# rmcar17/SpectralClusterSupertree

Hardware: AMD Instinct MI355X
Metric: top-level PCG build + Fiedler solve wall-time (s) at N taxa, 1/2/4/8 MI355X (lower is better)
Workload: dtype f64 (loop operator: fp32 image of W; fp64 renewal + confirmation)

## Files before the change

spectralclustersupertree_amd/csrc/scs_build.hip:

```cpp

#include <algorithm>

#include "scs_internal.h"

typedef unsigned long long u64;
typedef unsigned int u32;

constexpr u32 DEPTH_INF = 0xFFFFFFFFu;


__device__ __forceinline__ void rmq_offsets(int m, int a, int b, int (&o)[2]) {
    const int k = 31 - __clz(b - a);
    o[0] = k * m + a;
    o[1] = k * m + b - (1 << k);
}

template <typename K>
__device__ __forceinline__ K rmq_min(const K *__restrict__ base, int m, int a, int b) {
    int o[2];
    rmq_offsets(m, a, b, o);
    const K x = base[o[0]], y = base[o[1]];
    return x < y ? x : y;
}

// ... 1109 lines not shown
        SCS_HIP_CHECK(hipEventSynchronize(ev_x.b));
        SCS_HIP_CHECK(hipEventElapsedTime(&exch_ms, ev_x.a, ev_x.b));
        exch_bytes = (double)chunk_doubles * 8.0 * (world - 1);
    } else if (shared) {
        std::vector<int32_t> splits;
        SCS_TRY(scs_gather_row_splits(ctx, row_begin, row_end, n, splits));
        auto needs = [&](int dst, const int2 &t) {
            const int64_t lo = splits[dst], hi = splits[dst + 1];
            const int64_t r_lo = (int64_t)t.x * SCS_TR, r_hi = std::min<int64_t>(r_lo + SCS_TR, n);
            const int64_t c_lo = (int64_t)t.y * cols_per_tile, c_hi = std::min<int64_t>(c_lo + cols_per_tile, n);
            return (r_lo < hi && lo < r_hi) || (c_lo < hi && lo < c_hi);
        };
        std::vector<int64_t> send_off(world + 1, 0), recv_off(world + 1, 0);
        std::vector<int32_t> send_slots;
        std::vector<int2> recv_tiles;
        for (int p = 0; p < world; ++p) {
            for (size_t i = rank; i < all_tiles.size(); i += world)
                if (needs(p, all_tiles[i])) send_slots.push_back((int32_t)(i / world));
            send_off[p + 1] = (int64_t)send_slots.size() * SCS_TR * cols_per_tile;
            for (size_t i = p; i < all_tiles.size(); i += world)
                if (needs(rank, all_tiles[i])) recv_tiles.push_back(all_tiles[i]);
            recv_off[p + 1] = (int64_t)recv_tiles.size() * SCS_TR * cols_per_tile;
        }
        cached_buf d_send(ctx), d_recv(ctx);
        dev_buf d_slots(ctx), d_rtiles(ctx);
        SCS_TRY(d_send.alloc((size_t)send_off[world] * 8));
        SCS_TRY(d_recv.alloc((size_t)recv_off[world] * 8));
        SCS_TRY(d_slots.alloc(send_slots.size() * 4));
        SCS_TRY(d_rtiles.alloc(recv_tiles.size() * sizeof(int2)));
        ev_pair ev_x;
        SCS_TRY(ev_x.init());
        SCS_HIP_CHECK(hipEventRecord(ev_x.a, s));
        SCS_HIP_CHECK(hipMemcpyAsync(d_slots.p, send_slots.data(), send_slots.size() * 4,
                                     hipMemcpyHostToDevice, s));
        SCS_HIP_CHECK(hipMemcpyAsync(d_rtiles.p, recv_tiles.data(), recv_tiles.size() * sizeof(int2),
                                     hipMemcpyHostToDevice, s));
        if (!send_slots.empty())
            k_pack_tiles<<<(unsigned)send_slots.size(), 256, 0, s>>>(
                (const double *)d_tile_out.p, (const int32_t *)d_slots.p, cols_per_tile, (double *)d_send.p);
        SCS_HIP_CHECK(hipGetLastError());
        SCS_TRY(scs_comm_alltoallv_f64(&ctx->comm, (const double *)d_send.p, send_off.data(),
                                       (double *)d_recv.p, recv_off.data(), s));
        if (!recv_tiles.empty())
            k_unpack_received<<<(unsigned)recv_tiles.size(), cols_per_tile, 0, s>>>(
                (const double *)d_recv.p, (const int2 *)d_rtiles.p, n, row_begin, row_end, g->d_w,
                g->ld);
        SCS_HIP_CHECK(hipGetLastError());
        SCS_HIP_CHECK(hipEventRecord(ev_x.b, s));
        SCS_HIP_CHECK(hipEventSynchronize(ev_x.b));
        SCS_HIP_CHECK(hipEventElapsedTime(&exch_ms, ev_x.a, ev_x.b));
        exch_bytes = (double)(recv_off[world] - (recv_off[rank + 1] - recv_off[rank])) * 8.0;
    }
    SCS_HIP_CHECK(hipEventRecord(ev_total.b, s));
    SCS_HIP_CHECK(hipEventSynchronize(ev_total.b));
    h_off.in_flight = false;
    SCS_TRY(scs_tables_finish(ctx, tb));
    float total_ms = 0.f;
    SCS_HIP_CHECK(hipEventElapsedTime(&total_ms, ev_total.a, ev_total.b));
    if (n_batches == 1) {
        SCS_HIP_CHECK(hipEventElapsedTime(&prep_ms, ev_prep.a, ev_prep.b));
        SCS_HIP_CHECK(hipEventElapsedTime(&acc_ms, ev_acc.a, ev_acc.b));
        if (single_batch_spec) spec_ms = acc_ms;
    }

    if (stats) {
        memset(stats, 0, sizeof(*stats));
        stats->n_taxa = n;
        stats->n_trees = M;
        stats->row_begin = row_begin;
        stats->row_end = row_end;
        stats->symmetric = shared ? 2 : (sym ? 1 : 0);
        stats->exchange_ms = exch_ms;
        stats->exchange_bytes = exch_bytes;
        stats->n_tiles = (int32_t)tiles.size();
        stats->n_batches = n_batches;
        stats->spec_batches = spec_batches;
        stats->tree_parallel_batches = tree_par ? n_batches : 0;
        stats->spec_trees = spec_trees;
        stats->listed_batches = listed_batches;
        stats->prep_pieces = prep_pieces;
        stats->spec_ms = spec_ms;
        stats->cell_trees = (double)tiles.size() * SCS_TR * cols_per_tile * (double)M;
        stats->prep_ms = prep_ms;
        stats->accumulate_ms = acc_ms;
        stats->total_ms = total_ms;
        stats->bytes_w = 8.0 * rows * (double)n;
        stats->bytes_tables = 16.0 * (double)tb->n_leaves + 8.0 * M;
    }
    gd.g = nullptr;
    *out = g;
    return SCS_OK;
}

extern "C" int scs_graph_contract(scs_ctx *ctx, scs_graph *g, const int32_t *group_start,
                                  int32_t n_groups, scs_graph **out) {
    SCS_REQUIRE(ctx && g && group_start && out, "scs_graph_contract: null argument");
    if (g->mf) {
        scs_set_error("scs_graph_contract: a matrix-free graph has no matrix to contract");
        return SCS_EUNSUP;
    }
    if (g->upper) {
        scs_set_error("scs_graph_contract: an SCS_BUILD_UPPER graph holds no whole rows; build it "
                      "row-partitioned (SCS_BUILD_SHARED) when the node contracts");
        return SCS_EUNSUP;
    }
    SCS_REQUIRE(n_groups >= 1 && n_groups <= g->n, "scs_graph_contract: bad group count %d",
// ... 30 lines not shown
    if (e != hipSuccess) {
        scs_graph_free(ctx, ng);
        scs_set_error("scs_graph_contract: kernel failed: %s", hipGetErrorString(e));
        return SCS_EHIP;
    }
    scs_graph_free(ctx, g);
    *out = ng;
    return SCS_OK;
}

extern "C" int scs_graph_download_rows(scs_ctx *ctx, const scs_graph *g, int32_t first, int32_t count,
                                       double *out);

extern "C" int scs_graph_download(scs_ctx *ctx, const scs_graph *g, double *out) {
    SCS_REQUIRE(ctx && g && out, "scs_graph_download: null argument");
    SCS_REQUIRE(!g->mf, "scs_graph_download: a matrix-free graph has no matrix");
    SCS_HIP_CHECK(hipSetDevice(ctx->device));
    SCS_HIP_CHECK(hipStreamSynchronize(ctx->stream));
    const size_t rows = (size_t)(g->row_end - g->row_begin);
    if (g->upper) return scs_graph_download_rows(ctx, g, g->row_begin, (int32_t)rows, out);
    SCS_HIP_CHECK(hipMemcpy2D(out, (size_t)g->n * 8, g->d_w, (size_t)g->ld * 8, (size_t)g->n * 8,
                              rows, hipMemcpyDeviceToHost));
    return SCS_OK;
}

extern "C" int scs_graph_download_rows(scs_ctx *ctx, const scs_graph *g, int32_t first,
                                       int32_t count, double *out) {
    SCS_REQUIRE(ctx && g && out, "scs_graph_download_rows: null argument");
    SCS_REQUIRE(!g->mf, "scs_graph_download_rows: a matrix-free graph has no matrix");
    SCS_REQUIRE(count >= 1 && first >= g->row_begin && first + count <= g->row_end,
                "scs_graph_download_rows: rows [%d, %d) outside this rank's block [%d, %d)", first,
                first + count, g->row_begin, g->row_end);
    SCS_HIP_CHECK(hipSetDevice(ctx->device));
    SCS_HIP_CHECK(hipStreamSynchronize(ctx->stream));
    if (g->upper) {
        const size_t wcols = (size_t)(g->n - g->col0);
        for (int32_t i = 0; i < count; ++i) memset(out + (size_t)i * g->n, 0, (size_t)g->n * 8);
        SCS_HIP_CHECK(hipMemcpy2D(out + g->col0, (size_t)g->n * 8,
                                  g->d_w + (int64_t)(first - g->row_begin) * g->ld, (size_t)g->ld * 8,
                                  wcols * 8, (size_t)count, hipMemcpyDeviceToHost));
        for (int32_t i = 0; i < count; ++i) {
            const int32_t c0 = (first + i) / 256 * 256;
            if (c0 > g->col0) memset(out + (size_t)i * g->n + g->col0, 0, (size_t)(c0 - g->col0) * 8);
        }
        return SCS_OK;
    }
    SCS_HIP_CHECK(hipMemcpy2D(out, (size_t)g->n * 8, g->d_w + (int64_t)(first - g->row_begin) * g->ld,
                              (size_t)g->ld * 8, (size_t)g->n * 8, (size_t)count,
                              hipMemcpyDeviceToHost));
    return SCS_OK;
}

int scs_graph_prepare_degrees_begin(scs_ctx *ctx, scs_graph *g, bool want_w32) {
    if (g->deg_stage) return SCS_OK;
    const int n = g->n;
    const int rows = g->row_end - g->row_begin;
    if (g->mf && !g->have_deg) {
        SCS_HIP_CHECK(hipSetDevice(ctx->device));
        hipStream_t s = ctx->stream;
        if (!g->d_deg) SCS_TRY(scs_block_alloc(ctx, (size_t)n * 8, (void **)&g->d_deg));
        if (!g->d_dinv) SCS_TRY(scs_block_alloc(ctx, (size_t)n * 8, (void **)&g->d_dinv));
        SCS_TRY(scs_matfree_apply(ctx, g, nullptr, 0, 4, nullptr, s));
        k_dinv<<<(n + 255) / 256, 256, 0, s>>>(g->d_deg, n, g->d_dinv);
        SCS_HIP_CHECK(hipGetLastError());
        SCS_TRY(scs_pinned_get(ctx, (size_t)n * 8, &g->deg_stage));
        SCS_HIP_CHECK(hipMemcpyAsync(g->deg_stage, g->d_deg, (size_t)n * 8, hipMemcpyDeviceToHost, s));
        return SCS_OK;
    }
    const bool img_rows = ctx->comm.world > 1 && !g->upper;
    bool need_img = want_w32 && !g->have_w32 && !g->upper &&
                    (img_rows || (ctx->comm.world == 1 && g->row_begin == 0 && rows == n));
    if (g->have_deg && !need_img) return SCS_OK;
    SCS_HIP_CHECK(hipSetDevice(ctx->device));
    hipStream_t s = ctx->stream;
    if (need_img && !g->d_w32) {
        const size_t need = (size_t)rows * g->ld * 4;
        std::lock_guard<std::mutex> lock(ctx->cache_mu);
        if (ctx->w32_cache && ctx->w32_cache_bytes >= need) {
            g->d_w32 = ctx->w32_cache;
            g->w32_bytes = ctx->w32_cache_bytes;
            ctx->w32_cache = nullptr;
            ctx->w32_cache_bytes = 0;
        } else if (scs_dev_malloc(ctx, (void **)&g->d_w32, need) == hipSuccess) {
            g->w32_bytes = need;
            if (scs_dbg("SCS_TRACE_SOLVES") && atoi(scs_dbg("SCS_TRACE_SOLVES")))
                fprintf(stderr, "[image] hipMalloc of %.2f GB\n", need / 1073741824.0);
        } else {
            (void)hipGetLastError();
            g->d_w32 = nullptr;
            need_img = false;
        }
    }
    if (!need_img && g->have_deg) return SCS_OK;
    if (need_img && img_rows && g->have_deg) {
        dev_buf tmp(ctx);
        SCS_TRY(tmp.alloc((size_t)n * 8));
        k_degrees<true><<<(rows + 3) / 4, 256, 0, s>>>(g->d_w, g->ld, n, rows, g->row_begin, (double *)tmp.p, g->d_w32, 1);
        SCS_HIP_CHECK(hipGetLastError());
        SCS_HIP_CHECK(hipStreamSynchronize(s));
        g->have_w32 = true;
        return SCS_OK;
    }
    if (!g->d_deg) SCS_TRY(scs_block_alloc(ctx, (size_t)n * 8, (void **)&g->d_deg));
    if (!g->d_dinv) SCS_TRY(scs_block_alloc(ctx, (size_t)n * 8, (void **)&g->d_dinv));
    const int world = ctx->comm.world;
    if (need_img && !img_rows) {
        k_degrees<true><<<(rows + 3) / 4, 256, 0, s>>>(g->d_w, g->ld, n, rows, g->row_begin, g->d_deg, g->d_w32);
// ... 185 lines not shown
```

spectralclustersupertree_amd/csrc/scs_eig.hip:

```cpp

#include <algorithm>
#include <chrono>
#include <cmath>

#include "scs_internal.h"
#include "scs_policy.h"
#include "scs_symm.h"
#include "scs_matfree.h"
#include "scs_symm_tri.h"

#include <sched.h>
#include "scs_panel.h"

constexpr int MAXB = 16;
constexpr int MAXS = 64;
constexpr int SLD = MAXS + 1;

typedef double v4d __attribute__((ext_vector_type(4)));

__global__ void k_scale_rows(const double *__restrict__ x, int ldx, int c0, int b, int n,
                             const double *__restrict__ dinv, double *__restrict__ zt,
                             int64_t ldz) {
    const int idx = blockIdx.x * blockDim.x + threadIdx.x;
    if (idx >= n * b) return;
// ... 1595 lines not shown
        bool armed = false;
        double drop_tol = 0.0, seq = 0.0;
        double *report = nullptr;
    } tf1;
    dbuf coef1;
    bool use32 = false;
    bool gram_from32 = false;
    int n_apply32 = 0;
    std::vector<char> ev32;
    const double *fold_u = nullptr;
    int *fold_mask_r = nullptr;
    const double *fold_theta = nullptr;
    size_t ypart_cap = 0;
    int64_t chunk = 0;
    int gram_blocks = 0;
    std::vector<int32_t> splits;
    std::vector<hipEvent_t> ev;
    std::vector<hipEvent_t> ev_ag;
    hipEvent_t ev_cal[2] = {nullptr, nullptr};
    bool time_ag = false;
    int n_allgather = 0;
    int n_apply = 0;

    ~solver() {
        if (ctx) {
            ctx->event_pool.insert(ctx->event_pool.end(), ev.begin(), ev.end());
            ctx->event_pool.insert(ctx->event_pool.end(), ev_ag.begin(), ev_ag.end());
            for (auto e : ev_cal)
                if (e) ctx->event_pool.push_back(e);
        } else {
            for (auto e : ev_cal)
                if (e) hipEventDestroy(e);
            for (auto e : ev) hipEventDestroy(e);
            for (auto e : ev_ag) hipEventDestroy(e);
        }
    }
    int new_event(hipEvent_t *e) {
        if (ctx && !ctx->event_pool.empty()) {
            *e = ctx->event_pool.back();
            ctx->event_pool.pop_back();
            return SCS_OK;
        }
        SCS_HIP_CHECK(hipEventCreate(e));
        return SCS_OK;
    }

    double *small_at(int off) const { return small.d() + off; }

    void bind(scs_ctx *c, int n_, int b_ = 0, scs_graph *g_ = nullptr) {
        ctx = c;
        g = g_;
        s = c->stream;
        n = n_;
        b = b_;
        rows = g ? g->row_end - g->row_begin : 0;
        world = c->comm.world;
        gram_blocks = 256;
    }
    int team_splits() {
        SCS_TRY(scs_gather_row_splits(ctx, g->row_begin, g->row_end, g->n, splits));
        int max_rows = 0;
        for (int r = 0; r < world; ++r) max_rows = std::max(max_rows, splits[r + 1] - splits[r]);
        chunk = g->upper ? (int64_t)n * b : (int64_t)max_rows * b;
        return SCS_OK;
    }
    int team_buffers() {
        if (world == 1 || part_mode) return SCS_OK;
        SCS_TRY(yfull.alloc((size_t)n * b * 8));
        SCS_TRY(recv.alloc((size_t)chunk * world * 8));
        SCS_TRY(splits_d.alloc((size_t)(world + 1) * 4));
        SCS_HIP_CHECK(hipMemcpyAsync(splits_d.p, splits.data(), (size_t)(world + 1) * 4, hipMemcpyHostToDevice, s));
        return SCS_OK;
    }

    static bool image_layout(const scs_ctx *ctx, const scs_graph *g, int b) {
        const int world = ctx->comm.world;
        const bool one = world == 1 && !g->upper && g->row_begin == 0 && g->row_end == g->n;
        const bool row_ranks = world > 1 && !g->upper;
        return !g->mf && g->n >= 4096 && b == 4 && (one || row_ranks);
    }

    int gather(const double *send, double *recvb, size_t count) {
        hipEvent_t a = nullptr, b = nullptr;
        if (time_ag) {
            SCS_TRY(new_event(&a));
            SCS_TRY(new_event(&b));
            ev_ag.push_back(a);
            ev_ag.push_back(b);
            SCS_HIP_CHECK(hipEventRecord(a, s));
        }
        SCS_TRY(scs_comm_allgather_f64(&ctx->comm, send, recvb, count, s));
        if (time_ag) SCS_HIP_CHECK(hipEventRecord(b, s));
        ++n_allgather;
        return SCS_OK;
    }

    int last_nseg = 1;

    bool tri = false, part_mode = false;
    int tri_ct = 2, tri_nct = 0, tri_ntiles = 0;
    int tri_rb_lo = 0, tri_rb_hi = 0x7FFFFFFF;
    bool tri_backwards = false;
    dbuf tri_tiles, tri_pdir, tri_ptr, ysend;
    std::vector<int2> tiles_host;
    int tri32_nct = 0, tri32_ntiles = 0;
    double w32_bytes_per_apply = 0.0;
    int64_t ldz = 0;
    double w_bytes_per_apply = 0.0;

    int launch_symm_tri(const double *zin, double *yout) {
        const int tw = tri_ct * 128;
        const double *w_eff = g->d_w - (int64_t)g->row_begin * g->ld - g->col0;
        double *ptr_eff = tri_ptr.d() - (int64_t)tri_rb_lo * n * b;
        const int n_tf = panel_blocks16();
        const int ntiles = use32 ? tri32_ntiles : tri_ntiles;
#define TRI_T(B_, CT_, RPW_, D_, WT_, W_)                                                            \
    if (tf1.armed)                                                                                   \
        k_symm_tri_tf<B_, CT_, RPW_, D_, WT_><<<ntiles + n_tf, 256, 0, s>>>(                         \
            W_, g->ld, n, zin, ldz, tile_list, tri_pdir.d(), ptr_eff, n_tf, q.d(), fold_u,           \
            part.d(), n_tf, tf1.drop_tol, fold_mask_r, fold_theta, tf1.report, tf1.seq, part2.d(),   \
            coef1.d());                                                                              \
    else                                                                                             \
        k_symm_tri<B_, CT_, RPW_, D_, WT_><<<ntiles, 256, 0, s>>>(W_, g->ld, n, zin, ldz,            \
                                                                      tile_list, tri_pdir.d(), ptr_eff)
#define TRI(B_, CT_, RPW_, D_) TRI_T(B_, CT_, RPW_, D_, double, w_eff)
        const int2 *tile_list = (const int2 *)tri_tiles.p + (use32 ? 2 * tri_ntiles : 0) + (tri_backwards ? ntiles : 0);
        tri_backwards = !tri_backwards;
        if (use32) {
            TRI_T(4, 2, 2, 3, float, g->d_w32);
            ++n_apply32;
        } else if (b == 4) {
            if (tri_ct == 4) TRI(4, 4, 2, 3);
            else if (tri_ct == 1) TRI(4, 1, 4, 4);
            else TRI(4, 2, 4, 3);
        } else {
            if (tri_ct == 1) TRI(8, 1, 2, 6);
            else TRI(8, 2, 2, 4);
        }
#undef TRI
#undef TRI_T
        SCS_HIP_CHECK(hipGetLastError());
        tf1.armed = false;
        const bool img_tiles = use32;
        if (part_mode) {
            k_symm_tri_finish<<<(4 * n * b + 255) / 256, 256, 0, s>>>(tri_pdir.d(), ptr_eff, n, b, tw, tri_nct,
                                                                  nullptr, ysend.d(), tri_rb_lo, tri_rb_hi);
            SCS_HIP_CHECK(hipGetLastError());
            SCS_TRY(gather(ysend.d(), recv.d(), (size_t)n * b));
            if (yout) {
                k_sum_parts<<<(n * b + 255) / 256, 256, 0, s>>>(recv.d(), world, n, b, g->d_dinv, yout);
                SCS_HIP_CHECK(hipGetLastError());
            }
            last_nseg = world;
            return SCS_OK;
        }
        k_symm_tri_finish<<<(4 * n * b + 255) / 256, 256, 0, s>>>(tri_pdir.d(), tri_ptr.d(), n, b, img_tiles ? 512 : tw,
                                                              img_tiles ? tri32_nct : tri_nct,
                                                              yout ? g->d_dinv : nullptr,
                                                              yout ? yout : ypart.d());
        SCS_HIP_CHECK(hipGetLastError());
        last_nseg = 1;
        return SCS_OK;
    }
// ... 9 lines not shown
            return SCS_OK;
        }
        if (tri) return launch_symm_tri(zin, yout);
        const int64_t ld = g->ld;
        int rpw = 4, sdepth = 2;
        if (b == 16) rpw = 2;
        if (b == 4) sdepth = 4;
        const int rowblocks = (rows + 4 * rpw - 1) / (4 * rpw);
        const int n_macros = (int)(ld / (sdepth * SYMM_SUB));
        int nseg = (1024 + rowblocks - 1) / rowblocks;
        nseg = std::max(1, std::min(std::min(nseg, 4), n_macros));
        if (b == 8 && nseg < 2 && n_macros >= 2 && rowblocks < 2048) nseg = 2;
        const int mps = (n_macros + nseg - 1) / nseg;
        nseg = (n_macros + mps - 1) / mps;
        if (ypart_cap < (size_t)nseg * rows * b) {
            scs_set_error("internal: ypart buffer too small");
            return SCS_EINVAL;
        }
        dim3 grid((unsigned)rowblocks, (unsigned)nseg);
        switch (b) {
            case 4:
                if (use32) {
                    ++n_apply32;
                    k_symm<4, 4, 4, 3, float><<<grid, 256, 0, s>>>(g->d_w32, ld, rows, zin, ypart.d(), mps);
                } else {
                    k_symm<4, 4, 4, 3><<<grid, 256, 0, s>>>(g->d_w, ld, rows, zin, ypart.d(), mps);
                }
                break;
            case 8:
                k_symm<8, 4, 2, 2><<<grid, 256, 0, s>>>(g->d_w, ld, rows, zin, ypart.d(), mps);
                break;
            case 12:
                k_symm<12, 4, 2, 1><<<grid, 256, 0, s>>>(g->d_w, ld, rows, zin, ypart.d(), mps);
                break;
            case 16:
                k_symm<16, 2, 2, 2><<<grid, 256, 0, s>>>(g->d_w, ld, rows, zin, ypart.d(), mps);
                break;
            default:
                scs_set_error("unsupported block width %d (need 4, 8, 12 or 16)", b);
                return SCS_EUNSUP;
        }
        SCS_HIP_CHECK(hipGetLastError());
        last_nseg = nseg;
        if (yout)
            k_symm_finish<<<(rows * b + 255) / 256, 256, 0, s>>>(ypart.d(), nseg, rows, b,
                                                                 g->d_dinv, g->row_begin, yout);
        return SCS_OK;
    }

    int alloc_symm_buffers() {
        ypart_cap = (size_t)4 * rows * b;
        SCS_TRY(ypart.alloc(ypart_cap * 8));
        ldz = g->upper ? scs_round_up(n, SCS_LD_ALIGN) : g->ld;
        SCS_TRY(z.alloc((size_t)b * ldz * 8));
        SCS_HIP_CHECK(hipMemsetAsync(z.p, 0, (size_t)b * ldz * 8, s));
        w_bytes_per_apply = 8.0 * rows * (double)n;
        w32_bytes_per_apply = 4.0 * rows * (double)n;
        if (g->mf)
            w_bytes_per_apply = 2.0 * 16.0 * (double)g->mf->tb->n_leaves +
                                2.0 * 2.0 * 8.0 * (double)g->mf->tb->n_trees * (double)n * b;
        if (g->upper) {
            if (b != 4 && b != 8) {
                scs_set_error("an SCS_BUILD_UPPER graph is solved with block width 4 or 8 (asked: %d)", b);
                return SCS_EUNSUP;
            }
            tri = true;
            part_mode = true;
            tri_ct = 2;
            const int tw = 256;
            tri_nct = (n + tw - 1) / tw;
            tri_rb_lo = g->row_begin / TRI_TH;
            tri_rb_hi = (g->row_end + TRI_TH - 1) / TRI_TH;
            std::vector<int2> tiles;
            for (int i = tri_rb_lo; i < tri_rb_hi; ++i)
                for (int j = i * TRI_TH / tw; j < tri_nct; ++j) tiles.push_back(make_int2(i, j));
            tri_ntiles = (int)tiles.size();
            tiles.insert(tiles.end(), tiles.rbegin(), tiles.rend());
            SCS_TRY(tri_tiles.alloc(std::max<size_t>(tiles.size(), 1) * sizeof(int2)));
            SCS_HIP_CHECK(hipMemcpyAsync(tri_tiles.p, tiles.data(), tiles.size() * sizeof(int2),
                                         hipMemcpyHostToDevice, s));
            SCS_HIP_CHECK(hipStreamSynchronize(s));
            SCS_TRY(tri_pdir.alloc((size_t)tri_nct * n * b * 8));
            SCS_TRY(tri_ptr.alloc((size_t)(tri_rb_hi - tri_rb_lo) * n * b * 8));
            SCS_TRY(ysend.alloc((size_t)n * b * 8));
            if (!recv.p) SCS_TRY(recv.alloc((size_t)n * b * world * 8));
            w_bytes_per_apply = 8.0 * (double)tri_ntiles * TRI_TH * tw;
            return SCS_OK;
        }
        tri = !g->mf && world == 1 && rows == n && g->row_begin == 0 && n >= 4096 && (b == 4 || b == 8);
        if (tri) {
            const int tw = tri_ct * 128;
            const int n_rb = (n + TRI_TH - 1) / TRI_TH;
            tri_nct = (n + tw - 1) / tw;
            std::vector<int2> &tiles = tiles_host;
            tiles.clear();
            for (int i = 0; i < n_rb; ++i)
                for (int j = i * TRI_TH / tw; j < tri_nct; ++j) tiles.push_back(make_int2(i, j));
            tri_ntiles = (int)tiles.size();
            tiles.insert(tiles.end(), tiles.rbegin(), tiles.rend());
            {
                std::vector<int2> t32;
                tri32_nct = (n + 511) / 512;
                for (int i = 0; i < n_rb; ++i)
                    for (int j = i * TRI_TH / 512; j < tri32_nct; ++j) t32.push_back(make_int2(i, j));
                tri32_ntiles = (int)t32.size();
                tiles.insert(tiles.end(), t32.begin(), t32.end());
                tiles.insert(tiles.end(), t32.rbegin(), t32.rend());
                w32_bytes_per_apply = 4.0 * (double)tri32_ntiles * TRI_TH * 512;
            }
            SCS_TRY(tri_tiles.alloc(tiles.size() * sizeof(int2)));
            SCS_HIP_CHECK(hipMemcpyAsync(tri_tiles.p, tiles.data(), tiles.size() * sizeof(int2),
                                         hipMemcpyHostToDevice, s));
            SCS_TRY(tri_pdir.alloc((size_t)std::max(tri_nct, tri32_nct) * n * b * 8));
            SCS_TRY(tri_ptr.alloc((size_t)n_rb * n * b * 8));
            w_bytes_per_apply = 8.0 * (double)tri_ntiles * TRI_TH * tw;
        }
        return SCS_OK;
    }

    int timed_symm(bool timed, const double *zin, double *yout) {
        hipEvent_t e0 = nullptr, e1 = nullptr;
        if (timed) {
            SCS_TRY(new_event(&e0));
            SCS_TRY(new_event(&e1));
            ev.push_back(e0);
            ev.push_back(e1);
            ev32.push_back(use32 ? 1 : 0);
            SCS_HIP_CHECK(hipEventRecord(e0, s));
        }
        SCS_TRY(launch_symm(zin, yout));
        if (timed) SCS_HIP_CHECK(hipEventRecord(e1, s));
        ++n_apply;
        return SCS_OK;
    }

    int apply(const double *src, int c0s, double *dst, int c0d) {
        const int nb = n * b;
        k_scale_rows<<<(nb + 255) / 256, 256, 0, s>>>(src, 3 * b, c0s, b, n, g->d_dinv, z.d(),
                                                      ldz);
        SCS_TRY(timed_symm(true, z.d(), yloc.d()));
        const double *yf = yloc.d();
        if (part_mode) {
        } else if (world > 1) {
            SCS_TRY(gather(yloc.d(), recv.d(), (size_t)chunk));
            k_unpack<<<(nb + 255) / 256, 256, 0, s>>>(recv.d(), chunk, b,
                                                      (const int32_t *)splits_d.p, world, n,
                                                      yfull.d());
            yf = yfull.d();
        }
        k_store_cols<<<(nb + 255) / 256, 256, 0, s>>>(yf, b, n, dst, 3 * b, c0d);
        return SCS_OK;
    }

    int gram(const double *a, int lda, int ka, const double *bm, int ldb, int kb, double *out,
             bool mfma) {
        const int nout = ka * kb;
        int nparts;
        if (mfma && ka <= 48 && kb <= 48) {
            nparts = std::min(gram_blocks, std::max(1, (n + 3) / 4));
            const int ta = (ka + 15) / 16, tb = (kb + 15) / 16;
#define GM(TA, TB)                                                                               \
    if (ta == TA && tb == TB)                                                                    \
        k_gram_mfma<TA, TB><<<nparts, 64, 0, s>>>(a, lda, ka, bm, ldb, kb, n, part.d());
            GM(1, 1) GM(1, 2) GM(1, 3) GM(2, 1) GM(2, 2) GM(2, 3) GM(3, 1) GM(3, 2) GM(3, 3)
#undef GM
        } else {
            nparts = std::min(gram_blocks, std::max(1, (n + GRAM_CH - 1) / GRAM_CH));
            k_gram<<<nparts, 256, 0, s>>>(a, lda, ka, bm, ldb, kb, n, part.d());
        }
        k_reduce_partials<<<(nout + 3) / 4, 256, 0, s>>>(part.d(), nparts, nout, out);
        SCS_HIP_CHECK(hipGetLastError());
        return SCS_OK;
    }

    int update(double *y, int ldy, int kc, double alpha, const double *a, int lda, int ka,
               const double *c, int ldc, double sign) {
        k_update<<<(n + 15) / 16, 256, 0, s>>>(y, ldy, kc, alpha, a, lda, ka, c, ldc, sign, n);
        SCS_HIP_CHECK(hipGetLastError());
        return SCS_OK;
    }

    int rotate2(double *y, double *y2, int ld, int kc, const double *c, int ldc) {
        k_update<<<dim3((n + 15) / 16, 2), 256, 0, s>>>(y, ld, kc, 0.0, y, ld, kc, c, ldc, 1.0, n, y2, y2);
        SCS_HIP_CHECK(hipGetLastError());
        return SCS_OK;
    }

    static int panel_cap() {
        static const int cap = PANEL_BLOCKS_MAX;
        return cap;
    }
    int panel_blocks16() const { return std::max(1, std::min(panel_cap(), ((n + 15) / 16 + 3) / 4)); }
    int panel_blocks4() const { return std::max(1, std::min(panel_cap(), ((n + 3) / 4 + 3) / 4)); }

    template <int B>
    int fused_front(const double *uvec, const double *c, const double *d, const double *theta,
                    double *coef, int *mask_r, double drop_tol, double *report, double seq) {
        const int nb = panel_blocks16();
        k_panel_rr<B><<<nb, 256, 0, s>>>(q.d(), aq.d(), uvec, c, d, theta, n, part.d());
        k_small_orth<<<1, 256, 0, s>>>(part.d(), nb, B, drop_tol, coef, mask_r, theta, report, seq);
        k_panel_tf<B, true, false><<<nb, 256, 0, s>>>(q.d(), uvec, coef, n, part.d(), nullptr,
                                                      nullptr, 0);
        k_small_orth<<<1, 256, 0, s>>>(part.d(), nb, B, 0.0, coef, mask_r, theta, nullptr, 0.0);
// ... 69 lines not shown
        } else if (finish == 1) {
            GRAM_BACK(1);
        } else {
            GRAM_BACK(2);
        }
#undef GRAM_BACK
        time_ag = false;
        SCS_HIP_CHECK(hipGetLastError());
        return SCS_OK;
    }
};

constexpr int SM_G = 0;
constexpr int SM_T = SM_G + 48 * 48;
constexpr int SM_C = SM_T + 48 * 16;
constexpr int SM_D = SM_C + 48 * 16;
constexpr int SM_THETA = SM_D + 48 * 16;
constexpr int SM_RN = SM_THETA + 32;
constexpr int SM_MASK = SM_RN + 32;
constexpr int SM_TOTAL = SM_MASK + 32;

void sign_flip_and_store(const std::vector<double> &col0, const std::vector<double> &col1, int n,
                         double *maps) {
    for (int c = 0; c < 2; ++c) {
        const std::vector<double> &v = c == 0 ? col0 : col1;
        int arg = 0;
        double best = -1.0;
        for (int i = 0; i < n; ++i)
            if (std::fabs(v[i]) > best) {
                best = std::fabs(v[i]);
                arg = i;
            }
        const double sg = v[arg] < 0.0 ? -1.0 : 1.0;
        for (int i = 0; i < n; ++i) maps[(size_t)i * 2 + c] = sg * v[i];
    }
}

bool dbg_on(const char *name) {
    const char *e = scs_dbg(name);
    return e && atoi(e);
}
bool dbg_not_off(const char *name) {
    const char *e = scs_dbg(name);
    return !(e && !atoi(e));
}

struct loop_plan {
    const int lowp_mode = getenv("SCS_LOWP") ? atoi(getenv("SCS_LOWP")) : 2;
    const double lowp_max_bytes = getenv("SCS_LOWP_MAX_BYTES") ? atof(getenv("SCS_LOWP_MAX_BYTES")) : 16.0 * (1u << 30);
    const bool legacy_loop = dbg_on("SCS_LEGACY_LOOP");
    const bool split_small = dbg_on("SCS_SPLIT_SMALL");
    const bool fold_pass2_on = dbg_not_off("SCS_FOLD_PASS2"), overlap_pass1_on = dbg_not_off("SCS_OVERLAP_PASS1");
    const bool use_mfma = !dbg_on("SCS_NO_MFMA");

    bool fused(int b) const { return (b == 4 || b == 8) && !legacy_loop; }
    bool fold_pass2(int b) const { return fused(b) && !split_small && fold_pass2_on; }
    bool overlap_pass1(int b, bool tri, bool part_mode, int world) const {
        return fold_pass2(b) && tri && !part_mode && world == 1 && overlap_pass1_on;
    }
};

int choose_width(const scs_ctx *ctx, const scs_graph *g, int block, const loop_plan &plan, bool *want32) {
    const int n = g->n;
    const bool image_ok = solver::image_layout(ctx, g, 4) && plan.lowp_mode > 0 && plan.fold_pass2(4) &&
                          (g->have_w32 ||
                           4.0 * (double)(g->row_end - g->row_begin) * (double)g->ld <= plan.lowp_max_bytes);
    int b = block ? block : ((n >= 16384 && !image_ok) ? 8 : 4);
    if (g->upper && b > 8) b = 8;
    if (g->mf) b = std::min(b <= 4 ? 4 : 8, g->mf->b_cap);
    {
        const int allowed[] = {16, 12, 8, 4};
        const int cap = (n - 2) / 3;
        int pick = 4;
        for (int a : allowed)
            if (a <= b && a <= cap) {
                pick = a;
                break;
            }
        b = pick;
    }
    *want32 = image_ok && b == 4;
    return b;
}

struct lobpcg {
    scs_ctx *const ctx;
    scs_graph *const g;
    const hipStream_t s;
    const int n, b, q3;
    const loop_plan &plan;
    const bool fused;
    solver sv;
    scs_loop_policy policy;
    static constexpr double drop_tol = 1e-13;
    double *Q = nullptr, *AQ = nullptr, *X = nullptr, *R = nullptr, *AX = nullptr;
    double *G = nullptr, *T = nullptr, *C = nullptr, *D = nullptr, *TH = nullptr, *RN = nullptr;
    int *MASK = nullptr;
    bool constrained = false;
    int want = 0;
    const double *uvec = nullptr;
    dbuf x0d, res_part;
    int res_blocks = 0;
    std::vector<double> h_rn, h_th;
    double final_res[2] = {0.0, 0.0};
    double *qaq_out = nullptr;
    int rr_solve = 0, rr_parts = 0, mpar = 0;
    int *maskp[2] = {nullptr, nullptr};

    lobpcg(scs_ctx *ctx_, scs_graph *g_, int b_, const loop_plan &plan_)
        : ctx(ctx_), g(g_), s(ctx_->stream), n(g_->n), b(b_), q3(3 * b_), plan(plan_), fused(plan_.fused(b_)) {}

    int setup(double tol, bool want32) {
        sv.bind(ctx, n, b, g);
        sv.use_mfma = plan.use_mfma;
        SCS_TRY(sv.team_splits());
        SCS_TRY(sv.q.alloc((size_t)n * q3 * 8));
        SCS_TRY(sv.aq.alloc((size_t)n * q3 * 8));
        SCS_TRY(sv.alloc_symm_buffers());
        SCS_TRY(sv.yloc.alloc((size_t)sv.chunk * 8));
        SCS_TRY(sv.u.alloc((size_t)n * 8));
        SCS_TRY(sv.part.alloc((size_t)1024 * q3 * q3 * 8));
        SCS_TRY(sv.part2.alloc((size_t)1024 * q3 * q3 * 8));
        SCS_TRY(sv.part3.alloc((size_t)1024 * q3 * q3 * 8));
        SCS_TRY(sv.small.alloc((size_t)SM_TOTAL * 8));
        SCS_TRY(sv.team_buffers());
        SCS_HIP_CHECK(hipMemsetAsync(sv.q.p, 0, (size_t)n * q3 * 8, s));
        SCS_HIP_CHECK(hipMemsetAsync(sv.aq.p, 0, (size_t)n * q3 * 8, s));
        SCS_HIP_CHECK(hipMemsetAsync(sv.yloc.p, 0, (size_t)sv.chunk * 8, s));
        SCS_HIP_CHECK(hipMemsetAsync(sv.small.p, 0, (size_t)SM_TOTAL * 8, s));
        sv.fold_pass2 = plan.fold_pass2(b);
        sv.overlap_pass1 = plan.overlap_pass1(b, sv.tri, sv.part_mode, sv.world);

        Q = sv.q.d(), AQ = sv.aq.d();
        X = Q, R = Q + 2 * b;
        AX = AQ;
        G = sv.small_at(SM_G), T = sv.small_at(SM_T), C = sv.small_at(SM_C);
        D = sv.small_at(SM_D);
        TH = sv.small_at(SM_THETA), RN = sv.small_at(SM_RN);
        MASK = (int *)sv.small_at(SM_MASK);
        h_rn.resize(b);
        h_th.resize(b + 1);

        SCS_TRY(scs_graph_prepare_degrees(ctx, g));
        sv.use32 = want32 && g->have_w32;
        policy.tol = tol;
        policy.lowp_mode = plan.lowp_mode;
        policy.lowp_tol = 1e-8;
        policy.lowp_tol2 = 0.0;
        policy.lowp_state = sv.use32 ? 1 : 0;
        constrained = g->n_isolated == 0;
        want = constrained ? 1 : 2;
        return SCS_OK;
    }

    int project_u(double *Y, int passes) {
        if (!constrained) return SCS_OK;
        for (int pass = 0; pass < passes; ++pass) {
            SCS_TRY(sv.gram(sv.u.d(), 1, 1, Y, q3, b, C, false));
            SCS_TRY(sv.update(Y, q3, b, 1.0, sv.u.d(), 1, 1, C, b, -1.0));
        }
        return SCS_OK;
    }
    int svqb(double *Y, double *AY, int *mask_out) {
        for (int pass = 0; pass < 2; ++pass) {
            SCS_TRY(sv.gram(Y, q3, b, Y, q3, b, G, sv.use_mfma));
            k_small_svqb<<<1, 256, 0, s>>>(G, b, pass == 0 ? drop_tol : 0.0, T, mask_out);
            SCS_TRY(sv.update(Y, q3, b, 0.0, Y, q3, b, T, b, 1.0));
            if (AY) SCS_TRY(sv.update(AY, q3, b, 0.0, AY, q3, b, T, b, 1.0));
        }
        return SCS_OK;
    }
    int rotate_x() {
        SCS_TRY(sv.gram(X, q3, b, AX, q3, b, G, sv.use_mfma));
        k_small_rr_start<<<1, 256, 0, s>>>(G, b, MASK, T, D, TH, drop_tol);
        return sv.rotate2(X, AX, q3, b, T, b);
    }

    int start(const double *x_init) {
        if (x_init) {
            SCS_TRY(x0d.alloc((size_t)n * 8));
            SCS_HIP_CHECK(hipMemcpyAsync(x0d.p, x_init, (size_t)n * 8, hipMemcpyHostToDevice, s));
// ... 61 lines not shown
            if ((++spins & 0xFFFF) == 0) {
                const hipError_t qe = hipStreamQuery(s);
                if (qe != hipSuccess && qe != hipErrorNotReady) {
                    scs_set_error("scs_fiedler: stream failed: %s", hipGetErrorString(qe));
                    return SCS_EHIP;
                }
                if (qe == hipSuccess && hr[40] != seq) {
                    if (std::chrono::steady_clock::now() - t_wait > std::chrono::seconds(5)) {
                        scs_set_error("scs_fiedler: residual report lost at iteration %d", iter);
                        return SCS_EHIP;
                    }
                }
            }
        }
        for (int j = 0; j < b; ++j) h_rn[j] = hr[j];
        for (int j = 0; j <= b; ++j) h_th[j] = hr[16 + j];
        return SCS_OK;
    }

    int read_residual() {
        k_residual<<<res_blocks, 256, 0, s>>>(Q, AQ, b, TH, n, res_part.d());
        k_reduce_partials<<<(b + 3) / 4, 256, 0, s>>>(res_part.d(), res_blocks, b, RN);
        SCS_HIP_CHECK(hipMemcpyAsync(h_rn.data(), RN, (size_t)b * 8, hipMemcpyDeviceToHost, s));
        SCS_HIP_CHECK(hipMemcpyAsync(h_th.data(), TH, (size_t)(b + 1) * 8, hipMemcpyDeviceToHost, s));
        SCS_HIP_CHECK(hipStreamSynchronize(s));
        return SCS_OK;
    }
    double worst_residual() {
        double worst = 0.0;
        for (int j = 0; j < want; ++j) worst = std::max(worst, std::sqrt(h_rn[j]));
        for (int j = 0; j < want; ++j) final_res[constrained ? 1 : j] = std::sqrt(h_rn[j]);
        return worst;
    }

    int unfused_back() {
        SCS_TRY(project_u(R, 1));
        for (int pass = 0; pass < 2; ++pass) {
            SCS_TRY(sv.gram(Q, q3, 2 * b, R, q3, b, C, sv.use_mfma));
            SCS_TRY(sv.update(R, q3, b, 1.0, Q, q3, 2 * b, C, b, -1.0));
        }
        SCS_TRY(svqb(R, nullptr, MASK + 2 * b));
        SCS_TRY(sv.apply(Q, 2 * b, AQ, 2 * b));

        SCS_TRY(sv.gram(Q, q3, q3, AQ, q3, q3, G, sv.use_mfma));
        k_small_rr<<<1, 256, 0, s>>>(G, 0, q3, b, MASK, T, D, TH, MASK + b, drop_tol);
        k_rr_update<<<(n + 15) / 16, 256, 0, s>>>(Q, b, q3, T, D, n);
        k_rr_update<<<(n + 15) / 16, 256, 0, s>>>(AQ, b, q3, T, D, n);
        SCS_HIP_CHECK(hipGetLastError());
        return SCS_OK;
    }

    int renew() {
        sv.use32 = false;
        SCS_TRY(sv.apply(Q, 0, AQ, 0));
        SCS_TRY(sv.apply(Q, b, AQ, b));
        sv.use32 = policy.image_in_use();
        return SCS_OK;
    }

    int confirm(double tol, double *w2) {
        sv.use32 = false;
        SCS_TRY(sv.apply(Q, 0, AQ, 0));
        SCS_TRY(rotate_x());
        SCS_TRY(read_residual());
        *w2 = worst_residual();
        if (!(*w2 <= tol)) {
            SCS_TRY(svqb(X, AX, MASK));
            SCS_TRY(rotate_x());
            SCS_TRY(read_residual());
            *w2 = worst_residual();
        }
        return SCS_OK;
    }
    int restart_directions() {
        if (fused) k_unit_coeffs<<<(3 * b * b + 255) / 256, 256, 0, s>>>(T, D, b);
        rr_solve = 0;
        return SCS_OK;
    }

    int extract(hipEvent_t ev_b, double *maps_out, scs_stats *st) {
        hipEvent_t ev_c0 = nullptr, ev_c1 = nullptr;
        if (sv.new_event(&ev_c0) == SCS_OK && sv.new_event(&ev_c1) == SCS_OK) {
            sv.ev_cal[0] = ev_c0;
            sv.ev_cal[1] = ev_c1;
            hipEventRecord(ev_c0, s);
            hipEventRecord(ev_c1, s);
        }
        dbuf maps_d;
        SCS_TRY(maps_d.alloc((size_t)n * 2 * 8));
        k_extract_maps<<<(n + 255) / 256, 256, 0, s>>>(Q, q3, n, g->d_dinv, 1.0 / g->dd_norm, constrained ? 1 : 0,
                                                      maps_d.d());
        struct pinned_buf {
            scs_ctx *ctx;
            void *p = nullptr;
            ~pinned_buf() {
                if (p) scs_pinned_release(ctx, p);
            }
        } cols_h{ctx};
        SCS_TRY(scs_pinned_get(ctx, (size_t)n * 2 * 8, &cols_h.p));
        const double *cols = (const double *)cols_h.p;
        SCS_HIP_CHECK(hipMemcpyAsync(cols_h.p, maps_d.p, (size_t)n * 2 * 8, hipMemcpyDeviceToHost, s));
        if (!fused)
            SCS_HIP_CHECK(hipMemcpyAsync(h_th.data(), TH, (size_t)(b + 1) * 8, hipMemcpyDeviceToHost, s));
        SCS_HIP_CHECK(hipEventRecord(ev_b, s));
        SCS_HIP_CHECK(hipStreamSynchronize(s));
        std::vector<double> c0(n), c1(n);
        for (int i = 0; i < n; ++i) {
            c0[i] = cols[(size_t)i * 2];
// ... 12 lines not shown
        return SCS_OK;
    }

    void fill_stats(scs_stats *st) const {
        st->block = b;
        st->n_apply = sv.n_apply;
        st->n_apply32 = sv.n_apply32;
        st->used_constraint = constrained ? 1 : 0;
        st->resid[0] = final_res[0];
        st->resid[1] = final_res[1];
        double tot = 0.0, mn = 1e300, tot32 = 0.0;
        int n_timed = 0, n_timed32 = 0;
        for (size_t i = 0; i + 1 < sv.ev.size(); i += 2) {
            float t = 0.f;
            if (hipEventElapsedTime(&t, sv.ev[i], sv.ev[i + 1]) == hipSuccess) {
                if (i / 2 < sv.ev32.size() && sv.ev32[i / 2]) {
                    tot32 += t;
                    ++n_timed32;
                    continue;
                }
                tot += t;
                mn = std::min(mn, (double)t);
                ++n_timed;
            }
        }
        if (n_timed > 0) tot *= (double)(sv.n_apply - sv.n_apply32) / n_timed;
        if (n_timed32 > 0) tot32 *= (double)sv.n_apply32 / n_timed32;
        st->apply_ms_total = tot;
        st->apply32_ms_total = tot32;
        st->apply32_bytes = sv.n_apply32 ? sv.w32_bytes_per_apply + 8.0 * (double)n * b + 8.0 * (double)sv.rows * b : 0.0;
        st->apply_ms_min = n_timed ? mn : 0.0;
        {
            float t = 0.f;
            st->event_pair_ms = (sv.ev_cal[1] && hipEventElapsedTime(&t, sv.ev_cal[0], sv.ev_cal[1]) == hipSuccess) ? t : 0.0;
        }
        st->apply_bytes = sv.w_bytes_per_apply + 8.0 * (double)n * b + 8.0 * (double)sv.rows * b;
        {
            double ag = 0.0;
            int n_ag = 0;
            for (size_t i = 0; i + 1 < sv.ev_ag.size(); i += 2) {
                float t = 0.f;
                if (hipEventElapsedTime(&t, sv.ev_ag[i], sv.ev_ag[i + 1]) == hipSuccess) {
                    ag += t;
                    ++n_ag;
                }
            }
            st->n_allgather = sv.n_allgather;
            st->allgather_ms_total = n_ag ? ag * (double)sv.n_allgather / n_ag : 0.0;
            st->allgather_bytes = sv.world > 1 ? 8.0 * (double)sv.chunk * sv.world : 0.0;
        }
    }
};

}

static int fiedler_dense_onesided(scs_ctx *ctx, scs_graph *g, double *maps, scs_stats *st) {
    const int n = g->n;
    hipStream_t s = ctx->stream;
    SCS_REQUIRE(ctx->comm.world == 1 && !g->upper, "dense path needs the whole matrix on one rank (V = %d)", n);
    dbuf sd, wv, vv;
    SCS_TRY(sd.alloc((size_t)n * n * 8));
    SCS_TRY(wv.alloc(4 * 8));
    SCS_TRY(vv.alloc((size_t)n * 2 * 8));
    k_dense_s<<<(n * n + 255) / 256, 256, 0, s>>>(g->d_w, g->ld, n, g->d_dinv, sd.d());
    const size_t lds = (size_t)(n + (n & 1)) * DENSE2_LD * sizeof(double);
    SCS_HIP_CHECK(hipFuncSetAttribute((const void *)k_dense_onesided, hipFuncAttributeMaxDynamicSharedMemorySize,
                                      DENSE2_MAX * DENSE2_LD * (int)sizeof(double)));
    k_dense_onesided<<<1, 256, lds, s>>>(sd.d(), n, wv.d(), vv.d());
    SCS_HIP_CHECK(hipGetLastError());
    std::vector<double> w(4), v((size_t)n * 2), dinv(n);
    SCS_HIP_CHECK(hipMemcpyAsync(w.data(), wv.p, 4 * 8, hipMemcpyDeviceToHost, s));
    SCS_HIP_CHECK(hipMemcpyAsync(v.data(), vv.p, (size_t)n * 2 * 8, hipMemcpyDeviceToHost, s));
    SCS_HIP_CHECK(hipMemcpyAsync(dinv.data(), g->d_dinv, (size_t)n * 8, hipMemcpyDeviceToHost, s));
    SCS_HIP_CHECK(hipStreamSynchronize(s));
    std::vector<double> c0(n), c1(n);
    for (int i = 0; i < n; ++i) {
        c0[i] = v[(size_t)i * 2 + 0] * dinv[i];
        c1[i] = v[(size_t)i * 2 + 1] * dinv[i];
    }
    sign_flip_and_store(c0, c1, n, maps);
    if (st) {
        st->block = 0;
        st->converged = w[3] != 0.0 ? 1 : 0;
        st->lambda[0] = w[0];
        st->lambda[1] = w[1];
        st->lambda_next = w[2];
    }
    if (w[3] == 0.0) {
        scs_set_error("scs_fiedler: the dense one-sided Jacobi did not converge in 40 sweeps (V = %d)", n);
        return SCS_ENOCONV;
    }
    return SCS_OK;
}

static int fiedler_dense(scs_ctx *ctx, scs_graph *g, double *maps, scs_stats *st) {
    const int n = g->n;
    hipStream_t s = ctx->stream;
    SCS_REQUIRE(ctx->comm.world == 1, "dense small-V path needs world == 1 (V = %d)", n);
    dbuf sd, wv, vv;
    SCS_TRY(sd.alloc((size_t)n * n * 8));
    SCS_TRY(wv.alloc((size_t)n * 8));
    SCS_TRY(vv.alloc((size_t)n * n * 8));
    k_dense_s<<<(n * n + 255) / 256, 256, 0, s>>>(g->d_w, g->ld, n, g->d_dinv, sd.d());
    k_small_eig<<<1, 256, 0, s>>>(sd.d(), n, wv.d(), vv.d());
    std::vector<double> w(n), v((size_t)n * n), dinv(n);
    SCS_HIP_CHECK(hipMemcpyAsync(w.data(), wv.p, (size_t)n * 8, hipMemcpyDeviceToHost, s));
// ... 129 lines not shown
```

spectralclustersupertree_amd/csrc/scs_internal.h:

```cpp
#pragma once

#include <hip/hip_runtime.h>

#include <cstdarg>
#include <cstdint>
#include <cstdio>
#include <cstring>
#include <mutex>
#include <string>
#include <vector>

#include "../../include/scs_hip.h"

void scs_set_error(const char *fmt, ...);

#define SCS_HIP_CHECK(expr)                                                                  \
    do {                                                                                     \
        hipError_t e_ = (expr);                                                              \
        if (e_ != hipSuccess) {                                                              \
            scs_set_error("%s failed: %s (%s:%d)", #expr, hipGetErrorString(e_), __FILE__,   \
                          __LINE__);                                                         \
            return (e_ == hipErrorOutOfMemory) ? SCS_ENOMEM : SCS_EHIP;                      \
        }                                                                                    \
    } while (0)
// ... 162 lines not shown
    void *deg_stage = nullptr;
    float *d_w32 = nullptr;
    size_t w32_bytes = 0;
    bool have_w32 = false;
    double *d_deg = nullptr;
    double *d_dinv = nullptr;
    int32_t n_isolated = 0;
    double dd_norm = 0.0;
};

#include <memory>
struct forest_region {
    scs_ctx *ctx = nullptr;
    std::shared_ptr<forest_region> base;
    std::vector<void *> blocks;
    void *host_block = nullptr;
    ~forest_region() {
        for (void *p : blocks) scs_block_release(ctx, p);
        if (host_block) scs_pinned_release(ctx, host_block);
    }
    int alloc(size_t bytes, void **out) {
        SCS_TRY(scs_block_alloc(ctx, bytes, out));
        blocks.push_back(*out);
        return SCS_OK;
    }
};

struct scs_forest {
    int32_t n_taxa = 0, n_trees = 0;
    int64_t n_nodes = 0, n_leaves = 0;
    std::shared_ptr<forest_region> region;
    int64_t *node_off = nullptr;
    int32_t *parent = nullptr, *taxon = nullptr;
    double *length = nullptr, *support = nullptr;
    double *weights = nullptr;
    mutable int32_t *tree_id = nullptr;
    bool has_tables = false;
    int64_t *tree_off = nullptr;
    int32_t *leaf_taxon = nullptr, *adj_depth = nullptr, *tree_index = nullptr;
    double *adj_val = nullptr;
    unsigned char *present = nullptr;
    const int64_t *h_tree_off = nullptr;
    const int32_t *h_leaf_taxon = nullptr, *h_adj_depth = nullptr, *h_tree_index = nullptr;
    const double *h_adj_val = nullptr, *h_weights = nullptr;
    const unsigned char *h_present = nullptr;
};


int scs_graph_prepare_degrees(scs_ctx *ctx, scs_graph *g);
int scs_graph_prepare_degrees_begin(scs_ctx *ctx, scs_graph *g, bool want_w32 = false);
int scs_matfree_apply(scs_ctx *ctx, scs_graph *g, const double *zt, int64_t ldz, int b, double *y_out,
                      hipStream_t stream);
void scs_matfree_release(scs_graph *g);
int scs_gather_row_splits(scs_ctx *ctx, int32_t row_begin, int32_t row_end, int32_t n,
                          std::vector<int32_t> &splits);


static inline int64_t scs_round_up(int64_t x, int64_t m) { return (x + m - 1) / m * m; }
```

Before: 0.01400.

## Start degree prep before build sync and fuse renewal applies into one wide pass

Two ideas. First, on the single-device dense path, degree computation (and optionally the fp32 image of W) is enqueued right after the build's final event record, before the host synchronizes, so that work overlaps build teardown instead of running later in the Fiedler solve. Second, the fp64 renewal step, which applied the operator twice with block width 4, now runs a single apply at width 8 through the triangular symmetric kernel, so W is streamed once instead of twice. This costs larger z, yloc and tri scratch buffers, and adds coupling between build and eigensolver planning through a new helper.

```diff
diff --git a/spectralclustersupertree_amd/csrc/scs_build.hip b/spectralclustersupertree_amd/csrc/scs_build.hip
--- a/spectralclustersupertree_amd/csrc/scs_build.hip
+++ b/spectralclustersupertree_amd/csrc/scs_build.hip
@@ -1185,6 +1185,10 @@
         exch_bytes = (double)(recv_off[world] - (recv_off[rank + 1] - recv_off[rank])) * 8.0;
     }
     SCS_HIP_CHECK(hipEventRecord(ev_total.b, s));
+    if (!scatter) {
+        const int ahead = scs_fiedler_degrees_ahead(ctx, g);
+        if (ahead >= 0) SCS_TRY(scs_graph_prepare_degrees_begin(ctx, g, ahead == 1));
+    }
     SCS_HIP_CHECK(hipEventSynchronize(ev_total.b));
     h_off.in_flight = false;
     SCS_TRY(scs_tables_finish(ctx, tb));
@@ -1321,7 +1325,10 @@
 }
 
 int scs_graph_prepare_degrees_begin(scs_ctx *ctx, scs_graph *g, bool want_w32) {
-    if (g->deg_stage) return SCS_OK;
+    if (g->deg_stage) {
+        if (!want_w32 || g->have_w32) return SCS_OK;
+        SCS_TRY(scs_graph_prepare_degrees(ctx, g));
+    }
     const int n = g->n;
     const int rows = g->row_end - g->row_begin;
     if (g->mf && !g->have_deg) {
diff --git a/spectralclustersupertree_amd/csrc/scs_eig.hip b/spectralclustersupertree_amd/csrc/scs_eig.hip
--- a/spectralclustersupertree_amd/csrc/scs_eig.hip
+++ b/spectralclustersupertree_amd/csrc/scs_eig.hip
@@ -1671,7 +1671,7 @@
         g = g_;
         s = c->stream;
         n = n_;
-        b = b_;
+        b = bw = bl = b_;
         rows = g ? g->row_end - g->row_begin : 0;
         world = c->comm.world;
         gram_blocks = 256;
@@ -1715,6 +1715,8 @@
     }
 
     int last_nseg = 1;
+    bool want_wide = false;
+    int bw = 0, bl = 0;
 
     bool tri = false, part_mode = false;
     int tri_ct = 2, tri_nct = 0, tri_ntiles = 0;
@@ -1728,6 +1730,7 @@
     double w_bytes_per_apply = 0.0;
 
     int launch_symm_tri(const double *zin, double *yout) {
+        const int b = bl;
         const int tw = tri_ct * 128;
         const double *w_eff = g->d_w - (int64_t)g->row_begin * g->ld - g->col0;
         double *ptr_eff = tri_ptr.d() - (int64_t)tri_rb_lo * n * b;
@@ -1843,8 +1846,11 @@
         ypart_cap = (size_t)4 * rows * b;
         SCS_TRY(ypart.alloc(ypart_cap * 8));
         ldz = g->upper ? scs_round_up(n, SCS_LD_ALIGN) : g->ld;
-        SCS_TRY(z.alloc((size_t)b * ldz * 8));
-        SCS_HIP_CHECK(hipMemsetAsync(z.p, 0, (size_t)b * ldz * 8, s));
+        const bool tri_one = !g->upper && !g->mf && world == 1 && rows == n && g->row_begin == 0 && n >= 4096 && (b == 4 || b == 8);
+        bl = b;
+        bw = (want_wide && tri_one && b == 4 && tri_ct == 2) ? 8 : b;
+        SCS_TRY(z.alloc((size_t)bw * ldz * 8));
+        SCS_HIP_CHECK(hipMemsetAsync(z.p, 0, (size_t)bw * ldz * 8, s));
         w_bytes_per_apply = 8.0 * rows * (double)n;
         w32_bytes_per_apply = 4.0 * rows * (double)n;
         if (g->mf)
@@ -1878,7 +1884,7 @@
             w_bytes_per_apply = 8.0 * (double)tri_ntiles * TRI_TH * tw;
             return SCS_OK;
         }
-        tri = !g->mf && world == 1 && rows == n && g->row_begin == 0 && n >= 4096 && (b == 4 || b == 8);
+        tri = tri_one;
         if (tri) {
             const int tw = tri_ct * 128;
             const int n_rb = (n + TRI_TH - 1) / TRI_TH;
@@ -1902,8 +1908,8 @@
             SCS_TRY(tri_tiles.alloc(tiles.size() * sizeof(int2)));
             SCS_HIP_CHECK(hipMemcpyAsync(tri_tiles.p, tiles.data(), tiles.size() * sizeof(int2),
                                          hipMemcpyHostToDevice, s));
-            SCS_TRY(tri_pdir.alloc((size_t)std::max(tri_nct, tri32_nct) * n * b * 8));
-            SCS_TRY(tri_ptr.alloc((size_t)n_rb * n * b * 8));
+            SCS_TRY(tri_pdir.alloc((size_t)std::max(tri_nct, tri32_nct) * n * bw * 8));
+            SCS_TRY(tri_ptr.alloc((size_t)n_rb * n * bw * 8));
             w_bytes_per_apply = 8.0 * (double)tri_ntiles * TRI_TH * tw;
         }
         return SCS_OK;
@@ -1940,6 +1946,18 @@
             yf = yfull.d();
         }
         k_store_cols<<<(nb + 255) / 256, 256, 0, s>>>(yf, b, n, dst, 3 * b, c0d);
+        return SCS_OK;
+    }
+
+    int apply_wide(const double *src, int c0s, double *dst, int c0d) {
+        const int nb = n * bw;
+        k_scale_rows<<<(nb + 255) / 256, 256, 0, s>>>(src, 3 * b, c0s, bw, n, g->d_dinv, z.d(), ldz);
+        bl = bw;
+        const int rc = timed_symm(true, z.d(), yloc.d());
+        bl = b;
+        SCS_TRY(rc);
+        k_store_cols<<<(nb + 255) / 256, 256, 0, s>>>(yloc.d(), bw, n, dst, 3 * b, c0d);
+        SCS_HIP_CHECK(hipGetLastError());
         return SCS_OK;
     }
 
@@ -2115,6 +2133,8 @@
     const bool split_small = dbg_on("SCS_SPLIT_SMALL");
     const bool fold_pass2_on = dbg_not_off("SCS_FOLD_PASS2"), overlap_pass1_on = dbg_not_off("SCS_OVERLAP_PASS1");
     const bool use_mfma = !dbg_on("SCS_NO_MFMA");
+    const bool degrees_ahead = dbg_not_off("SCS_DEGREES_AHEAD");
+    const bool renew_wide = dbg_not_off("SCS_RENEW_WIDE");
 
     bool fused(int b) const { return (b == 4 || b == 8) && !legacy_loop; }
     bool fold_pass2(int b) const { return fused(b) && !split_small && fold_pass2_on; }
@@ -2179,8 +2199,10 @@
         SCS_TRY(sv.team_splits());
         SCS_TRY(sv.q.alloc((size_t)n * q3 * 8));
         SCS_TRY(sv.aq.alloc((size_t)n * q3 * 8));
+        sv.want_wide = plan.renew_wide;
         SCS_TRY(sv.alloc_symm_buffers());
-        SCS_TRY(sv.yloc.alloc((size_t)sv.chunk * 8));
+        const size_t yloc_len = std::max((size_t)sv.chunk, (size_t)n * sv.bw);
+        SCS_TRY(sv.yloc.alloc(yloc_len * 8));
         SCS_TRY(sv.u.alloc((size_t)n * 8));
         SCS_TRY(sv.part.alloc((size_t)1024 * q3 * q3 * 8));
         SCS_TRY(sv.part2.alloc((size_t)1024 * q3 * q3 * 8));
@@ -2189,7 +2211,7 @@
         SCS_TRY(sv.team_buffers());
         SCS_HIP_CHECK(hipMemsetAsync(sv.q.p, 0, (size_t)n * q3 * 8, s));
         SCS_HIP_CHECK(hipMemsetAsync(sv.aq.p, 0, (size_t)n * q3 * 8, s));
-        SCS_HIP_CHECK(hipMemsetAsync(sv.yloc.p, 0, (size_t)sv.chunk * 8, s));
+        SCS_HIP_CHECK(hipMemsetAsync(sv.yloc.p, 0, yloc_len * 8, s));
         SCS_HIP_CHECK(hipMemsetAsync(sv.small.p, 0, (size_t)SM_TOTAL * 8, s));
         sv.fold_pass2 = plan.fold_pass2(b);
         sv.overlap_pass1 = plan.overlap_pass1(b, sv.tri, sv.part_mode, sv.world);
@@ -2357,8 +2379,12 @@
 
     int renew() {
         sv.use32 = false;
-        SCS_TRY(sv.apply(Q, 0, AQ, 0));
-        SCS_TRY(sv.apply(Q, b, AQ, b));
+        if (sv.bw == 2 * b) {
+            SCS_TRY(sv.apply_wide(Q, 0, AQ, 0));
+        } else {
+            SCS_TRY(sv.apply(Q, 0, AQ, 0));
+            SCS_TRY(sv.apply(Q, b, AQ, b));
+        }
         sv.use32 = policy.image_in_use();
         return SCS_OK;
     }
@@ -2477,6 +2503,16 @@
     }
 };
 
+}
+
+int scs_fiedler_degrees_ahead(const scs_ctx *ctx, const scs_graph *g) {
+    if (ctx->comm.world != 1 || g->upper || g->mf || g->n <= DENSE2_MAX) return -1;
+    if (g->row_begin != 0 || g->row_end != g->n) return -1;
+    const loop_plan plan{};
+    if (!plan.degrees_ahead) return -1;
+    bool want32 = false;
+    (void)choose_width(ctx, g, 0, plan, &want32);
+    return want32 ? 1 : 0;
 }
 
 static int fiedler_dense_onesided(scs_ctx *ctx, scs_graph *g, double *maps, scs_stats *st) {
diff --git a/spectralclustersupertree_amd/csrc/scs_internal.h b/spectralclustersupertree_amd/csrc/scs_internal.h
--- a/spectralclustersupertree_amd/csrc/scs_internal.h
+++ b/spectralclustersupertree_amd/csrc/scs_internal.h
@@ -238,6 +238,7 @@
 int scs_matfree_apply(scs_ctx *ctx, scs_graph *g, const double *zt, int64_t ldz, int b, double *y_out,
                       hipStream_t stream);
 void scs_matfree_release(scs_graph *g);
+int scs_fiedler_degrees_ahead(const scs_ctx *ctx, const scs_graph *g);
 int scs_gather_row_splits(scs_ctx *ctx, int32_t row_begin, int32_t row_end, int32_t n,
                           std::vector<int32_t> &splits);
 
```

Result: no change. 0.01380 (median of 2 runs) (-1.5%).
